# MartinBeseda/FEM-ElastoPlasticity

Hardware: AMD Instinct MI355X
Metric: element*quadpt updates/sec (return-map + K_tan assemble) (higher is better)
Workload: dtype f64; 1 GPU; Plasticity2D_DP strip-footing square, 708x708 cells = 1002528 P1 elements per GPU (BASELINE configs[3]), Drucker-Prager, strain->return map->K_tan CSR values->F per step; element_type=P1, points_per_gpu=1002528, points_total=1002528, elements_total=1002528, nnz_per_gpu=14052388, smooth_points=178150, apex_points=573758, state=bands, route=node, elements_per_gpu=1002528, parallelism=single GPU

## Files before the change

### fem-elastoplasticity_amd/csrc/fep_api.hip

```cpp
#include "fep_common.h"
#include "fep_host.h"
#include "fep_kernels.hip.h"
#include "fep_staging.h"

#include <algorithm>
#include <chrono>
#include <cstdio>
#include <cstdlib>
#include <cstring>
#include <map>
#include <mutex>
#include <new>
#include <thread>
#include <vector>

using namespace fep;

#ifndef FEP_P4_TPB
#define FEP_P4_TPB 256
#define FEP_P4_JS 1
#endif

thread_local int fep_g_last_hip = 0;
#define g_last_hip fep_g_last_hip
// ... 27 lines not shown
    uint16_t *pt_codes = nullptr, *pt_fcodes = nullptr;
    uint4 *pt_fix = nullptr, *pt_ffix = nullptr;
    uint2* pt_fixT = nullptr;
    int64_t n_patch = 0;
#ifdef FEP_ABLATION
    unsigned long long* phase_clk = nullptr;
#endif
    double *Pc = nullptr, *Pf = nullptr;
    bool elem_geo = true;
    MatU matu{};
    int32_t* elem = nullptr;
    double *coords = nullptr, *dh1 = nullptr, *dh2 = nullptr, *wf = nullptr;
    double *dphi1 = nullptr, *dphi2 = nullptr, *weight = nullptr, *det = nullptr;
    double *shear = nullptr, *bulk = nullptr, *eta = nullptr, *c = nullptr;
    int32_t *segptr = nullptr, *perm = nullptr, *iptr = nullptr, *ilist = nullptr;
    uint32_t* meta = nullptr;
    bool p1_lds = false;
    double *geo = nullptr, *xy = nullptr;
    P1Tab p1tab{};
    int32_t *perm2 = nullptr, *ncol = nullptr;
    int32_t *wg_elist = nullptr, *wg_rng = nullptr;
    bool p1_rng = false, p1_pk = false;
    uint2* pk = nullptr;
    int4* tdesc = nullptr;
    int32_t* tstart = nullptr;
    int n_wg_p1 = 0;
    bool p1_fused = false, p1_fused_rng = false;
    bool asm_from_nodes = false;
    bool p1_dma = false;
    int fused_mode = 1;
    int lds_NL = 0;
    int32_t *wg_nlist = nullptr, *wg_nrng = nullptr;
    uint32_t* el_nodes = nullptr;
    unsigned long long* slot_counts = nullptr;
    bool has_orphans = false;
    uint16_t* perm_l = nullptr;
    int tile = 256;
    int gn_tile = 256;
    size_t gn_lds = 0;
    int lds_L = 0, lds_C = 0;
    double *Kc = nullptr, *fe = nullptr;
    double *s_int = nullptr, *ds_int = nullptr;
    uint2* blk_counts = nullptr;
    int n_count_blocks = 0;
    void* hbuf[12] = {};
    size_t hbuf_bytes[12] = {};
    std::vector<int32_t> indptr, indices;
    bool profiling = false;
    std::vector<hipEvent_t> events;
    bool verbose = false;
};

__attribute__((visibility("hidden"))) int fep_set_device(int dev) {
    int n = 0;
    hipError_t e = hipGetDeviceCount(&n);
    if (e != hipSuccess || n <= 0) { g_last_hip = (int)e; (void)hipGetLastError(); return FEP_ENODEV; }
    if (dev < 0 || dev >= n) return FEP_ENODEV;
    e = hipSetDevice(dev);
    if (e != hipSuccess) { g_last_hip = (int)e; (void)hipGetLastError(); return FEP_ENODEV; }
    return FEP_OK;
}

template <class T> static int dmalloc(fep_ctx* c, T** p, int64_t count) {
    *p = nullptr;
    if (count <= 0) count = 1;
    try { c->owned.reserve(c->owned.size() + 1); } catch (...) { return FEP_ENOMEM; }
// ... 353 lines not shown
    fep_ctx* c = nullptr;
    int r;
    try {
        r = ctx_create_impl(c, ctx_out, device_id, elem_type, n_e, n_n, elements_h, coords_h, dhatp1_h, dhatp2_h, wf_h);
    } catch (const std::bad_alloc&) {
        r = FEP_ENOMEM;
    } catch (...) {
        r = FEP_EINVAL;
    }
    if (r != FEP_OK) { if (c) fep_ctx_destroy(c); *ctx_out = nullptr; }
    return r;
}

struct MeshIn {
    const Symbolic& S;
    const int32_t* elem;
    const double *coords, *dh1, *dh2, *wf;
    bool validate;
};

static int setup_p1_node(fep_ctx* c, const MeshIn& in, bool* taken) {
    *taken = false;
    fep_host::P1Options opt;
#ifdef FEP_ABLATION
    if (const char* tl = fep_tune("FEP_P1_TILE")) c->tile = std::atoi(tl) == 128 ? 128 : 256;
    {
        const char* pth = fep_tune("FEP_P1_PATH");
        auto is = [&](const char* v) { return pth && std::strcmp(pth, v) == 0; };
        opt.allow_lds = !is("node_direct");
        opt.allow_rng = !is("node_list");
        opt.allow_pk = !is("node_unpacked");
        opt.allow_fused = !is("node2k");
        if (const char* sg = fep_tune("FEP_P1_SEGS")) opt.max_segs = std::max(1, std::min(std::atoi(sg), fep_host::kSegMax));
    }
#endif
    opt.tile = c->tile;
    fep_host::P1Plan P;
    FEP_TRY(fep_host::build_p1_plan(in.S, c->n_e, c->n_n, in.elem, opt, P));
    if (in.validate) {
        const int bad = fep_host::validate_p1_plan(P, in.S, c->n_e, c->n_n, in.elem);
        if (bad) { std::fprintf(stderr, "[fep] P1 plan fails check %d\n", bad); return FEP_EINVAL; }
    }
#ifndef FEP_ABLATION
    if (!(P.lds && P.pk)) {
        if (c->verbose) std::fprintf(stderr, "[fep] P1 plan without the LDS-staged packed form (lds %d pk %d): element route\n", (int)P.lds, (int)P.pk);
        return FEP_OK;
    }
#endif
    *taken = true;
    c->n_wg_p1 = (int)P.n_wg;
    c->p1_lds = P.lds; c->lds_L = P.L; c->lds_C = P.C; c->p1_rng = P.rng; c->p1_pk = P.pk;
    c->p1_fused = P.fused; c->p1_fused_rng = P.fused_rng; c->lds_NL = P.NL;
#ifdef FEP_ABLATION
    if (const char* am = fep_tune("FEP_P1_ASM")) c->asm_from_nodes = std::strcmp(am, "nodes") == 0;
    if (const char* dm = fep_tune("FEP_P1_DMA")) c->p1_dma = std::strcmp(dm, "0") != 0;
    if (const char* fm = fep_tune("FEP_P1_FUSED"))
        c->fused_mode = std::strcmp(fm, "off") == 0 ? 0 : std::strcmp(fm, "kf") == 0 ? 1 : 2;
#endif
    FEP_TRY(upload(c, &c->perm2, P.perm2.data(), (int64_t)P.perm2.size()));
    FEP_TRY(upload(c, &c->ncol, in.S.ncol.data(), (int64_t)in.S.ncol.size()));
    FEP_TRY(upload(c, &c->tdesc, (const int4*)P.tdesc.data(), (int64_t)P.tdesc.size() / 4));
    if (P.lds) {
        FEP_TRY(upload(c, &c->wg_elist, P.elist_pad.data(), (int64_t)P.elist_pad.size()));
        FEP_TRY(upload(c, &c->perm_l, P.codes_pad.data(), (int64_t)P.codes_pad.size()));
        if (P.rng) FEP_TRY(upload(c, &c->wg_rng, P.rng_tab.data(), (int64_t)P.rng_tab.size()));
        if (P.pk) FEP_TRY(upload(c, &c->pk, (const uint2*)P.pkv.data(), (int64_t)P.pkv.size()));
    }
    if (P.fused) {
        FEP_TRY(upload(c, &c->el_nodes, P.elnodes.data(), (int64_t)P.elnodes.size()));
        if (P.fused_rng) FEP_TRY(upload(c, &c->wg_nrng, P.nrng_tab.data(), (int64_t)P.nrng_tab.size()));
        else FEP_TRY(upload(c, &c->wg_nlist, P.nlist_pad.data(), (int64_t)P.nlist_pad.size()));
        FEP_TRY(dmalloc(c, &c->slot_counts, 256 * 16));
        HIP_TRY(hipMemset(c->slot_counts, 0, 256 * 16 * sizeof(unsigned long long)));
    }
    if (c->verbose)
        std::fprintf(stderr, "[fep] P1 plan: %lld tiles of <= %d blocks in <= %d segment(s), staged elements %lld "
                     "(%.2f per element, <= %d per tile), staged nodes <= %d, codes <= %d; lds %d rng %d pk %d fused %d/%d\n",
                     (long long)P.n_wg, P.tile, P.n_segs, (long long)P.staged_total, (double)P.staged_total / (double)c->n_e,
                     P.L, P.NL, P.C, (int)P.lds, (int)P.rng, (int)P.pk, (int)P.fused, (int)P.fused_rng);
    FEP_TRY(dmalloc(c, &c->geo, 6 * c->n_e));
    for (int a = 0; a < 3; ++a) { c->p1tab.h1[a] = in.dh1[a]; c->p1tab.h2[a] = in.dh2[a]; }
    c->p1tab.wf = in.wf[0];
    c->n_count_blocks = (int)grid_for(c->n_e, kBlock);
    return FEP_OK;
}

#ifdef FEP_ABLATION
static int setup_gen_node(fep_ctx* c, const MeshIn& in, bool* taken) {
    fep_host::GnPlan G;
    fep_host::build_gn_plan(in.S, c->n_p, c->n_q, c->n_e, G);
    *taken = G.ok;
    if (!G.ok) return FEP_OK;
    c->gn_tile = G.tile; c->lds_L = G.L; c->lds_C = G.C; c->gn_lds = G.lds;
    FEP_TRY(upload(c, &c->wg_elist, G.elist_pad.data(), (int64_t)G.elist_pad.size()));
    FEP_TRY(upload(c, &c->perm_l, G.codes_pad.data(), (int64_t)G.codes_pad.size()));
    FEP_TRY(upload(c, &c->ncol, in.S.ncol.data(), (int64_t)in.S.ncol.size()));
    c->n_count_blocks = (int)grid_for(c->n_int, kBlock);
    return FEP_OK;
}
#endif

static void elem_form(fep_ctx* c, bool patch_form) {
    c->elem_geo = elem_geo_default(c->elem_type, patch_form);
#ifdef FEP_ABLATION
    if (const char* ge = fep_tune("FEP_ELEM_GEO")) c->elem_geo = std::strcmp(ge, "0") != 0;
    if (const char* lp = fep_tune("FEP_ELEM_LDS_PAD")) c->lds_pad = std::max(0, std::atoi(lp));
#endif
}

static int setup_patch(fep_ctx* c, const MeshIn& in, bool* taken) {
    *taken = false;
    elem_form(c, true);
// ... 366 lines not shown
}

static int launch_force(fep_ctx* c, hipStream_t st, double* f_out) {
    hipLaunchKernelGGL(force_reduce_kernel, dim3(grid_for(c->n_n, kBlock)), dim3(kBlock), 0, st,
                       c->n_n, c->iptr, c->ilist, c->fe, f_out);
    HIP_TRY(hipGetLastError());
    return FEP_OK;
}

static int launch_fixup(fep_ctx* c, hipStream_t st, double* k_data, double* f_out, unsigned long long* counts_d, bool* counted) {
    const unsigned nb_k = k_data ? grid_for(c->n_open, kBlock) : 0u;
    const unsigned nb_f = f_out ? grid_for(c->n_fopen, kBlock) : 0u;
    const unsigned grid = nb_k + nb_f + (counts_d ? 1u : 0u);
    if (grid == 0) return FEP_OK;
    hipLaunchKernelGGL(fixup_kernel, dim3(grid), dim3(kBlock), 0, st, (int)nb_k, c->n_open, c->pt_fix, c->pt_fixT, c->n_fopen, c->pt_ffix,
                       c->pt_plist, c->Pc, c->Pf, k_data, f_out, c->n_count_blocks, c->blk_counts, counts_d);
    HIP_TRY(hipGetLastError());
    *counted = counts_d != nullptr;
    return FEP_OK;
}

static int launch_p1_node(fep_ctx* c, hipStream_t st, const double* ds, const double* s, double* k_data, double* f_out,
                          unsigned long long* counts_d, bool* counted) {
    if (!((k_data && ds) || (f_out && s))) return FEP_OK;
    if (!k_data) ds = nullptr;
    if (!f_out) s = nullptr;
    const int n_wg = c->n_wg_p1;
    const unsigned grid = 8 * ((n_wg + 7) / 8);
#ifdef FEP_ABLATION
    if (c->p1_fused && c->asm_from_nodes) {
        const size_t lds_stage = (((size_t)c->lds_L * 15 * sizeof(double) + (size_t)c->lds_C * 2 + 15) & ~(size_t)15) +
                                 (size_t)c->lds_NL * 2 * sizeof(double2);
        const size_t lds = std::max(lds_stage, (size_t)c->tile * 3 * sizeof(double2));
        if (c->lds_L > 256 || c->lds_NL > 256) return FEP_ESTATE;
        FEP_TRY(with_bool(c->p1_fused_rng, [&](auto rng) {
            return launch_lds(p1_fused_kernel<false, 256, decltype(rng)::value, 1, 1, true>, grid, 256, lds, kLdsDefault, st,
                              c->n_e, c->lds_L, c->lds_C, c->lds_NL, c->perm_l, c->wg_elist, (const int4*)c->wg_rng,
                              c->wg_nlist, (const int4*)c->wg_nrng, c->el_nodes, c->pk, c->tdesc, c->xy, c->p1tab,
                              (const double*)nullptr, make_e0(nullptr), (const double*)nullptr, c->shear, c->bulk, c->eta,
                              c->c, c->matu, (double*)nullptr, (double*)nullptr, (double*)nullptr, (uint8_t*)nullptr,
                              k_data, f_out, n_wg, (unsigned long long*)nullptr, ds, s, c->n_count_blocks, c->blk_counts, counts_d);
        }));
        *counted = counts_d != nullptr;
        return FEP_OK;
    }
    if (!c->p1_lds) {
        hipLaunchKernelGGL(p1_node_kernel, dim3(grid_for(c->n_blk, kBlock)), dim3(kBlock), 0, st,
                           c->n_blk, c->n_e, c->segptr, c->perm2, c->meta, c->ncol, c->geo, ds, s, k_data, f_out);
        HIP_TRY(hipGetLastError());
        return FEP_OK;
    }
#else
    if (!c->p1_lds) return FEP_ESTATE;
#endif
    const size_t lds = std::max((size_t)c->lds_L * 15 * sizeof(double) + (size_t)c->lds_C * sizeof(uint16_t),
                                (size_t)c->tile * 3 * sizeof(double2));
    if (c->verbose) {
        static bool once = false;
        if (!once) {
            once = true;
            std::fprintf(stderr, "[fep] p1 assembly kernel: %d tiles of <= %d blocks, staged elements <= %d, codes <= %d, "
                         "LDS %zu bytes per workgroup\n", n_wg, c->tile, c->lds_L, c->lds_C, lds);
        }
    }
    FEP_TRY(with_ablation_bool<false>(c->tile == 128, [&](auto t128) {
        constexpr int TPB = decltype(t128)::value ? 128 : 256;
        if (c->lds_L > TPB) return FEP_ESTATE;
        return with_bool(c->p1_rng, [&](auto rng) {
            return with_ablation_bool<true>(c->p1_pk, [&](auto pk) {
                return launch_lds(p1_node_lds_kernel<TPB, decltype(rng)::value, 1, decltype(pk)::value>, grid, TPB, lds,
                                  kLdsDefault, st, c->n_e, c->lds_L, c->lds_C, c->segptr, c->perm_l, c->meta, c->ncol,
// ... 31 lines not shown
    FEP_TRY(with_type(c->elem_type, [&](auto et) {
        using ET = decltype(et);
        if constexpr (ET::type == FEP_P1 || ET::type == FEP_P4) return FEP_EINVAL;
        else return with_bool(c->gn_tile == 256, [&](auto t256) {
            constexpr int TPB = decltype(t256)::value ? 256 : 128;
            return launch_lds(node_lds_kernel<ET::NP, ET::NQ, TPB>, grid, TPB, c->gn_lds, kLdsNodeLds, st, c->n_blk, c->n_e,
                              c->lds_L, c->lds_C, c->segptr, c->perm_l, c->meta, c->ncol, c->wg_elist, c->elem, c->xy,
                              c->dh1, c->dh2, c->wf, k_data ? ds : nullptr, f_out ? s : nullptr, k_data, f_out, n_wg,
                              c->n_count_blocks, c->blk_counts, counts_d);
        });
    }));
    *counted = counts_d != nullptr;
    return FEP_OK;
}
#endif

static int launch_p1_fused(fep_ctx* c, hipStream_t st, const double* u, E0 e0, const double* ep, double* eout, double* s,
                           double* ds, uint8_t* indp, double* k_data, double* f_out, unsigned long long* counts_d) {
    const bool dma = c->p1_dma;
    const size_t Cp = dma ? ((size_t)c->lds_C + 127) & ~(size_t)127 : (size_t)c->lds_C;
    const size_t NLp = dma ? ((size_t)c->lds_NL + 63) & ~(size_t)63 : (size_t)c->lds_NL;
    const size_t lds_stage = (((size_t)c->lds_L * 15 * sizeof(double) + Cp * 2 + 15) & ~(size_t)15) + NLp * 2 * sizeof(double2);
    const size_t lds = std::max(lds_stage, (size_t)c->tile * 3 * sizeof(double2));
    const int n_wg = c->n_wg_p1;
    const unsigned grid = 8 * ((n_wg + 7) / 8);
    if (c->lds_L > c->tile || c->lds_NL > c->tile) return FEP_ESTATE;
    const bool full = eout || s || ds || indp;
    FEP_TRY(with_ablation_bool<false>(full, [&](auto full_c) {
        return with_bool(c->p1_fused_rng, [&](auto rng) {
            return with_ablation_bool<false>(dma, [&](auto dma_c) {
                return with_ablation_bool<false>(c->tile == 128, [&](auto t128) {
                    constexpr int TPB = decltype(t128)::value ? 128 : 256;
                    return launch_lds(p1_fused_kernel<decltype(full_c)::value, TPB, decltype(rng)::value, 1, 1, false, decltype(dma_c)::value>,
                                      grid, TPB, lds, kLdsDefault, st, c->n_e, c->lds_L, c->lds_C, c->lds_NL, c->perm_l,
                                      c->wg_elist, (const int4*)c->wg_rng, c->wg_nlist, (const int4*)c->wg_nrng, c->el_nodes,
                                      c->pk, c->tdesc, c->xy, c->p1tab, u, e0, ep, c->shear, c->bulk, c->eta, c->c, c->matu,
                                      eout, s, ds, indp, k_data, f_out, n_wg,
                                      counts_d ? c->slot_counts : (unsigned long long*)nullptr, (const double*)nullptr,
                                      (const double*)nullptr, 0, (const uint2*)nullptr, (unsigned long long*)nullptr);
                });
            });
        });
    }));
    if (counts_d) {
        hipLaunchKernelGGL(counts_finalize_kernel, dim3(1), dim3(256), 0, st, c->slot_counts, counts_d);
        HIP_TRY(hipGetLastError());
    }
    return FEP_OK;
}

static int launch_assembly(fep_ctx* c, hipStream_t st, const double* ds, const double* s, double* k_data, double* f_out,
                           unsigned long long* counts_d, bool* counted, bool* f_due) {
    *counted = *f_due = false;
    if (c->route == Route::P1Node) return launch_p1_node(c, st, ds, s, k_data, f_out, counts_d, counted);
#ifdef FEP_ABLATION
    if (c->route == Route::GenNode) return launch_gn_node(c, st, ds, s, k_data, f_out, counts_d, counted);
#endif
    if (c->route == Route::Patch) return launch_fixup(c, st, k_data, f_out, counts_d, counted);
    return launch_reduce(c, st, k_data, f_out, counts_d, counted, f_due);
}

extern "C" int fep_step_dev(fep_ctx* c, void* stream, const double* u_d, const double* e0_h,
                            double* ep_prev_d, int accept, double* e_out_d, double* s_d, double* ds_d,
                            uint8_t* ind_p_d, double* k_data_d, double* f_out_d, int64_t* counts_d) {
    if (!c || !u_d) return FEP_EINVAL;
    if (!fep_aligned16(u_d) || !fep_aligned16(f_out_d) || !fep_aligned16(k_data_d)) return FEP_EINVAL;
    if (!c->have_materials) return FEP_ESTATE;
    FEP_TRY(fep_set_device(c->device));
    hipStream_t st = (hipStream_t)stream;
// ... 384 lines not shown
```

### fem-elastoplasticity_amd/csrc/fep_host.h

```cpp
#pragma once
#include <algorithm>
#include <atomic>
#include <cstdint>
#include <cstdlib>
#include <cstring>
#include <exception>
#include <new>
#include <system_error>
#include <thread>
#include <utility>
#include <vector>

#include "../../include/fep.h"

namespace fep_host {

struct U2 { uint32_t x, y; };

inline int worker_count() {
    if (const char* e = std::getenv("FEP_HOST_THREADS")) { const int v = std::atoi(e); if (v >= 1) return std::min(v, 64); }
    return (int)std::max(1u, std::min(16u, std::thread::hardware_concurrency()));
}

template <class F> void parallel_chunks(int64_t n, F&& f) {
    const int nw = (int)std::max<int64_t>(1, std::min<int64_t>(worker_count(), n));
    std::vector<std::thread> th;
    th.reserve(nw);
    std::vector<int> inline_chunks;
    std::vector<std::exception_ptr> err((size_t)nw);
    auto guarded = [&f, &err](int64_t lo, int64_t hi, int w) {
        try { f(lo, hi, w); } catch (...) { err[(size_t)w] = std::current_exception(); }
    };
    for (int w = 1; w < nw; ++w) {
        const int64_t lo = n * w / nw, hi = n * (w + 1) / nw;
        try { th.emplace_back([&guarded, lo, hi, w]() { guarded(lo, hi, w); }); }
        catch (const std::system_error&) { inline_chunks.push_back(w); }
    }
    guarded(0, n / nw, 0);
    for (int w : inline_chunks) guarded(n * w / nw, n * (w + 1) / nw, w);
    for (auto& t : th) t.join();
    for (const std::exception_ptr& e : err)
        if (e) std::rethrow_exception(e);
// ... 67 lines not shown
                    const int64_t blk = S.nptr[n] + slot;
                    S.ncol[blk] = buf[i].first;
                    S.meta[blk] = ((uint32_t)deg[n] << 16) | (buf[i].first == (int32_t)n ? 0x8000u : 0u) | (uint32_t)slot;
                    S.segptr[blk] = (int32_t)pos;
                }
                S.perm[pos++] = buf[i].second;
            }
        }
    });
    S.segptr[n_blk] = (int32_t)n_contrib;
    return FEP_OK;
}

inline int row_tiles(const Symbolic& S, int64_t n_n, int tile, std::vector<int32_t>& tstart) {
    tstart.assign(1, 0);
    for (int64_t n = 0, cur = 0; n < n_n; ++n) {
        const int64_t d = S.nptr[n + 1] - S.nptr[n];
        if (d > tile) return FEP_ERANGE;
        if (cur + d > tile) { tstart.push_back(S.nptr[n]); cur = 0; }
        cur += d;
    }
    tstart.push_back(S.nptr[n_n]);
    return FEP_OK;
}

constexpr int kSegMax = 4;
constexpr int kDescInts = 4 * (1 + kSegMax);

struct P1Options {
    int tile = 256;
    int max_segs = 2;
    int staged_cap = 128;
    bool allow_lds = true, allow_rng = true, allow_pk = true, allow_fused = true;
};

struct P1Plan {
    int tile = 256, n_segs = 1;
    int64_t n_wg = 0, staged_total = 0, staged_nodes_total = 0;
    std::vector<int32_t> tdesc;
    std::vector<int32_t> perm2;
    bool lds = false, rng = false, pk = false, fused = false, fused_rng = false;
    int L = 0, C = 0, NL = 0;
    std::vector<int32_t> elist_pad, rng_tab, nlist_pad, nrng_tab;
    std::vector<uint16_t> codes_pad;
    std::vector<U2> pkv;
    std::vector<uint32_t> elnodes;
};

struct Tile { int nseg = 0; int32_t fb[kSegMax] = {}, nb[kSegMax] = {}, fn[kSegMax] = {}, nn[kSegMax] = {}; };

inline int make_tiles(const Symbolic& S, int64_t n_n, int tile, int max_segs, std::vector<Tile>& tiles) {
    tiles.clear();
    max_segs = std::max(1, std::min(max_segs, kSegMax));
    std::vector<uint8_t> assigned((size_t)n_n, 0);
    for (int64_t n = 0; n < n_n; ++n) assigned[n] = S.nptr[n + 1] == S.nptr[n];
    std::vector<int32_t> nbrs;
    int64_t p = 0;
    while (true) {
        while (p < n_n && assigned[p]) ++p;
        if (p >= n_n) break;
        Tile t;
        int total_nodes = 0, total_blocks = 0;
        int64_t start = p;
        for (int s = 0; s < max_segs; ++s) {
            const int seg_budget = std::min((tile - total_blocks + (max_segs - s) - 1) / (max_segs - s),
                                            max_segs > 1 ? tile / max_segs + 8 : tile);
            int64_t n = start;
            int blocks = 0;
            while (n < n_n && !assigned[n] && blocks + (S.nptr[n + 1] - S.nptr[n]) <= seg_budget && total_nodes + (int)(n - start) < 255) {
                blocks += S.nptr[n + 1] - S.nptr[n];
                ++n;
            }
            if (n == start) {
                if (s > 0) break;
                if (S.nptr[n + 1] - S.nptr[n] > tile) return FEP_ERANGE;
                blocks = S.nptr[n + 1] - S.nptr[n];
                ++n;
            }
            t.fb[s] = S.nptr[start]; t.nb[s] = blocks; t.fn[s] = (int32_t)start; t.nn[s] = (int32_t)(n - start);
// ... 9 lines not shown
            nbrs.erase(std::unique(nbrs.begin(), nbrs.end()), nbrs.end());
            size_t best = 0, best_len = 0;
            for (size_t i = 0; i < nbrs.size();) {
                size_t j = i + 1;
                while (j < nbrs.size() && nbrs[j] == nbrs[j - 1] + 1) ++j;
                if (j - i > best_len) { best_len = j - i; best = i; }
                i = j;
            }
            if (best_len < 2) break;
            start = nbrs[best];
            {
                int64_t lo = start;
                int gap = 0;
                while (lo > 0 && !assigned[lo - 1] && gap < 32) { --lo; ++gap; }
                if (gap < 32) start = lo;
            }
        }
        tiles.push_back(t);
    }
    return FEP_OK;
}

inline void runs_of(const std::vector<int32_t>& l, int32_t* d , bool& fits) {
    int nr = 0, cum = 0;
    for (size_t i = 0; i < l.size();) {
        size_t j = i + 1;
        while (j < l.size() && l[j] == l[j - 1] + 1) ++j;
        if (nr == 8) { fits = false; break; }
        cum += (int)(j - i);
        d[2 * nr] = l[i]; d[2 * nr + 1] = cum;
        ++nr; i = j;
    }
    for (; nr < 8; ++nr) { d[2 * nr] = l.empty() ? 0 : l[0]; d[2 * nr + 1] = cum; }
}

inline int build_p1_plan_segs(const Symbolic& S, int64_t n_e, int64_t n_n, const int32_t* elem, const P1Options& opt,
                              int max_segs, P1Plan& P) {
    P = P1Plan();
    P.tile = opt.tile;
    const int TILE = opt.tile;
    if (n_e >= (int64_t)1 << 27) return FEP_ERANGE;
    const int64_t n_blk = (int64_t)S.ncol.size();
    P.perm2.resize(S.perm.size());
    for (size_t i = 0; i < S.perm.size(); ++i) {
        const int64_t code = S.perm[i];
        const int64_t ab = code / n_e, e = code - ab * n_e;
        P.perm2[i] = (int32_t)((e << 4) | ((ab / 3) << 2) | (ab % 3));
    }
    std::vector<Tile> tiles;
    const int r = make_tiles(S, n_n, TILE, max_segs, tiles);
    if (r != FEP_OK) return r;
    if (max_segs > 1 && opt.staged_cap > 0) {
        std::vector<int32_t> count(tiles.size(), 0);
        parallel_chunks((int64_t)tiles.size(), [&](int64_t lo, int64_t hi, int) {
            std::vector<int32_t> l;
            for (int64_t g = lo; g < hi; ++g) {
                const Tile& t = tiles[g];
                if (t.nseg < 2) continue;
                l.clear();
                for (int s = 0; s < t.nseg; ++s)
                    for (int32_t c = S.segptr[t.fb[s]]; c < S.segptr[t.fb[s] + t.nb[s]]; ++c) l.push_back(P.perm2[c] >> 4);
                std::sort(l.begin(), l.end());
                count[g] = (int32_t)(std::unique(l.begin(), l.end()) - l.begin());
            }
        });
        std::vector<Tile> split;
// ... 112 lines not shown
                const int32_t* d = P.tdesc.data() + g * kDescInts;
                const int nb = d[1];
                if (d[2] > 255) { pk_bad[g] = 1; continue; }
                order.resize(nb); blk.resize(nb); node_of.resize(nb); off.resize(nb);
                int k = 0, node_base = 0, o = 0;
                for (int s = 0; s < t.nseg; ++s) {
                    for (int32_t n = t.fn[s]; n < t.fn[s] + t.nn[s]; ++n)
                        for (int32_t b = S.nptr[n]; b < S.nptr[n + 1]; ++b) {
                            blk[k] = b; node_of[k] = node_base + (n - t.fn[s]); off[k] = o;
                            o += S.segptr[b + 1] - S.segptr[b];
                            ++k;
                        }
                    node_base += t.nn[s];
                }
                if (k != nb) { pk_bad[g] = 1; continue; }
                for (int i = 0; i < nb; ++i) order[i] = i;
                std::stable_sort(order.begin(), order.end(), [&](int x, int y) {
                    return S.segptr[blk[x] + 1] - S.segptr[blk[x]] > S.segptr[blk[y] + 1] - S.segptr[blk[y]];
                });
                for (int lane = 0; lane < nb; ++lane) {
                    const int kk = order[lane];
                    const int32_t b = blk[kk];
                    const uint32_t mt = S.meta[b];
                    const uint32_t len = (uint32_t)(S.segptr[b + 1] - S.segptr[b]), deg = mt >> 16, slot = mt & 0x7fffu;
                    const uint32_t diag = (mt >> 15) & 1u;
                    if (len > 15 || deg > 255 || slot > 255 || off[kk] > 2047) { pk_bad[g] = 1; break; }
                    P.pkv[(size_t)d[0] + lane] = U2{(uint32_t)off[kk] | (len << 11) | (deg << 15) | (slot << 23) | (diag << 31),
                                                    (uint32_t)kk | ((uint32_t)node_of[kk] << 8)};
                }
            }
        });
    for (int64_t g = 0; g < n_wg && pk_ok; ++g) pk_ok = !pk_bad[g];
    P.pk = pk_ok;
    if (!pk_ok) { P.pkv.clear(); return FEP_OK; }
    if (!opt.allow_fused) return FEP_OK;
    std::vector<std::vector<int32_t>> nlists(n_wg);
    P.elnodes.assign((size_t)(n_wg * LP), 0u);
    std::vector<uint8_t> nbad((size_t)n_wg, 0);
    parallel_chunks(n_wg, [&](int64_t lo, int64_t hi, int) {
        for (int64_t g = lo; g < hi; ++g) {
            const std::vector<int32_t>& l = lists[g];
            std::vector<int32_t>& nl = nlists[g];
            nl.reserve(3 * l.size());
            for (int32_t e : l)
                for (int a = 0; a < 3; ++a) nl.push_back(elem[(int64_t)a * n_e + e]);
            std::sort(nl.begin(), nl.end());
            nl.erase(std::unique(nl.begin(), nl.end()), nl.end());
            if (nl.size() > 1023) { nbad[g] = 1; continue; }
            for (size_t i = 0; i < l.size(); ++i) {
                uint32_t word = 0u;
                for (int a = 0; a < 3; ++a) {
                    const int32_t nd = elem[(int64_t)a * n_e + l[i]];
                    word |= (uint32_t)(std::lower_bound(nl.begin(), nl.end(), nd) - nl.begin()) << (10 * a);
                }
                P.elnodes[(size_t)(g * LP) + i] = word;
            }
            for (size_t i = l.size(); i < (size_t)LP; ++i) P.elnodes[(size_t)(g * LP) + i] = P.elnodes[(size_t)(g * LP)];
        }
    });
    size_t nlmax = 0;
    for (int64_t g = 0; g < n_wg; ++g) {
        if (nbad[g]) { P.elnodes.clear(); return FEP_OK; }
        nlmax = std::max(nlmax, nlists[g].size());
        P.staged_nodes_total += (int64_t)nlists[g].size();
    }
    if (nlmax == 0 || nlmax > (size_t)TILE) { P.elnodes.clear(); return FEP_OK; }
    for (int64_t g = 0; g < n_wg; ++g) {
        for (int32_t i = 0; i < n_own[g]; ++i) P.elnodes[(size_t)(g * LP) + i] |= 1u << 30;
        P.tdesc[(size_t)g * kDescInts + 2] |= n_own[g] << 8;
    }
    const int64_t NLP = (int64_t)((nlmax + 1) & ~(size_t)1);
    P.NL = (int)NLP;
    P.nlist_pad.assign((size_t)(n_wg * NLP), 0);
    P.nrng_tab.assign((size_t)n_wg * 16, 0);
    bool nfits = P.rng;
    for (int64_t g = 0; g < n_wg; ++g) {
        const std::vector<int32_t>& nl = nlists[g];
        std::fill(P.nlist_pad.begin() + g * NLP, P.nlist_pad.begin() + (g + 1) * NLP, nl[0]);
        std::copy(nl.begin(), nl.end(), P.nlist_pad.begin() + g * NLP);
        if (nfits) runs_of(nl, P.nrng_tab.data() + g * 16, nfits);
    }
    for (int64_t g = 0; g < n_wg; ++g) P.tdesc[(size_t)g * kDescInts + 3] |= (int32_t)(nlists[g].size() << 16);
    P.fused_rng = nfits;
    const size_t lds_f = (((size_t)P.L * 15 * sizeof(double) + (size_t)P.C * 2 + 15) & ~(size_t)15) + (size_t)NLP * 32;
    P.fused = lds_f <= 96 * 1024;
    if (!P.fused) P.elnodes.clear();
    return FEP_OK;
}

inline int build_p1_plan(const Symbolic& S, int64_t n_e, int64_t n_n, const int32_t* elem, const P1Options& opt, P1Plan& P) {
    int r = build_p1_plan_segs(S, n_e, n_n, elem, opt, 1, P);
    if (r != FEP_OK || opt.max_segs <= 1 || !P.lds || !P.pk) return r;
    P1Plan Q;
    r = build_p1_plan_segs(S, n_e, n_n, elem, opt, opt.max_segs, Q);
    if (r == FEP_OK && Q.lds && Q.pk && (Q.fused || !P.fused) && (Q.rng || !P.rng) && (Q.fused_rng || !P.fused_rng) &&
        Q.staged_total * 100 <= P.staged_total * 95) P = std::move(Q);
    return FEP_OK;
}

inline int validate_p1_plan(const P1Plan& P, const Symbolic& S, int64_t n_e, int64_t n_n, const int32_t* elem) {
    const int64_t n_blk = (int64_t)S.ncol.size();
    if ((int64_t)P.tdesc.size() != P.n_wg * kDescInts) return 1;
    std::vector<uint8_t> seen((size_t)n_blk, 0);
    std::vector<int> owners((size_t)n_e, 0);
    int64_t pk_base = 0;
    for (int64_t g = 0; g < P.n_wg; ++g) {
        const int32_t* d = P.tdesc.data() + g * kDescInts;
        const int nseg = d[3] & 15, n_staged = (d[3] >> 4) & 4095, n_staged_nodes = (d[3] >> 16) & 4095;
        const int nn_desc = d[2] & 255, n_own = d[2] >> 8;
        if (d[0] != pk_base || nseg < 1 || nseg > kSegMax || d[1] > P.tile || d[1] < 1 || n_own > n_staged) return 2;
        int nb = 0, nn = 0;
        for (int s = 0; s < nseg; ++s) {
            const int32_t fb = d[4 + 4 * s], sb = d[5 + 4 * s], fn = d[6 + 4 * s], sn = d[7 + 4 * s];
            if (fn < 0 || fn + sn > n_n || sn < 1 || S.nptr[fn] != fb || S.nptr[fn + sn] != fb + sb) return 3;
            for (int32_t b = fb; b < fb + sb; ++b) { if (seen[b]) return 4; seen[b] = 1; }
            nb += sb; nn += sn;
        }
        if (nb != d[1] || nn != nn_desc) return 5;
        pk_base += nb;
        if (!P.lds) continue;
        const int32_t* el = P.elist_pad.data() + g * P.L;
        const int n_list = n_staged;
        if (n_list < 1 || n_list > P.L) return 18;
        for (int i = 0; i < P.L; ++i) {
            if (el[i] < 0 || el[i] >= n_e) return 6;
            if (i >= n_list && el[i] != el[0]) return 18;
        }
        {
            std::vector<int32_t> srt(el, el + n_list);
            std::sort(srt.begin(), srt.end());
            if (std::adjacent_find(srt.begin(), srt.end()) != srt.end()) return 18;
            if (P.fused)
                for (int i = 1; i < n_list; ++i)
                    if (i != n_own && el[i] <= el[i - 1]) return 18;
        }
        if (P.rng) {
            const int32_t* r = P.rng_tab.data() + g * 16;
            for (int i = 0; i < P.L; ++i) {
                int e = r[0] + i;
                for (int k = 1; k < 8; ++k) e = i >= r[2 * k - 1] ? r[2 * k] + (i - r[2 * k - 1]) : e;
                e = i < r[15] ? e : r[0];
                if (e != el[i]) return 7;
            }
// ... 2 lines not shown
            std::vector<uint8_t> lane_blk((size_t)nb, 0);
            for (int lane = 0; lane < nb; ++lane) {
                const U2 w = P.pkv[(size_t)d[0] + lane];
                const int beg = (int)(w.x & 2047u), len = (int)((w.x >> 11) & 15u), deg = (int)((w.x >> 15) & 255u);
                const int slot = (int)((w.x >> 23) & 255u), blk = (int)(w.y & 255u), nod = (int)((w.y >> 8) & 255u);
                if (beg + len > P.C || blk >= nb || nod >= nn || lane_blk[blk]) return 8;
                lane_blk[blk] = 1;
                const int rel = 4 * blk - 2 * slot;
                if (rel < 0 || (rel >> 1) + deg + 1 > 2 * nb || slot >= deg) return 9;
                for (int c = beg; c < beg + len; ++c) {
                    const unsigned code = P.codes_pad[(size_t)g * P.C + c];
                    if ((int)(code >> 4) >= n_list || ((code >> 2) & 3) > 2 || (code & 3) > 2) return 10;
                }
            }
        }
        if (P.fused) {
            const int32_t* nl = P.nlist_pad.data() + g * P.NL;
            int n_nl = 1;
            for (int i = 0; i < P.NL; ++i) {
                if (nl[i] < 0 || nl[i] >= n_n) return 11;
                if (i > 0 && nl[i] > nl[i - 1]) n_nl = i + 1;
            }
            if (n_nl != n_staged_nodes) return 19;
            if (P.fused_rng) {
                const int32_t* r = P.nrng_tab.data() + g * 16;
                for (int i = 0; i < P.NL; ++i) {
                    int n = r[0] + i;
                    for (int k = 1; k < 8; ++k) n = i >= r[2 * k - 1] ? r[2 * k] + (i - r[2 * k - 1]) : n;
                    n = i < r[15] ? n : r[0];
                    if (n != nl[i]) return 12;
                }
            }
            for (int i = 0; i < P.L; ++i) {
                const uint32_t w = P.elnodes[(size_t)g * P.L + i];
                for (int a = 0; a < 3; ++a) {
                    const int loc = (int)((w >> (10 * a)) & 1023u);
                    if (loc >= P.NL || nl[loc] != elem[(int64_t)a * n_e + el[i]]) return 13;
                }
                if (((w >> 30) & 1u) != (i < n_own ? 1u : 0u)) return 14;
                if (i < n_own) owners[el[i]]++;
            }
        }
    }
    if (pk_base != n_blk) return 15;
    for (int64_t b = 0; b < n_blk; ++b) if (!seen[b]) return 16;
    if (P.fused) for (int64_t e = 0; e < n_e; ++e) if (owners[e] != 1) return 17;
    return 0;
}

struct GnPlan {
    bool ok = false;
    int tile = 256, L = 0, C = 0;
    size_t lds = 0;
    std::vector<int32_t> elist_pad;
    std::vector<uint16_t> codes_pad;
};

inline void build_gn_plan(const Symbolic& S, int n_p, int n_q, int64_t n_e, GnPlan& G) {
    const int64_t n_blk = (int64_t)S.ncol.size();
    for (int TILE : {256, 128}) {
        const int64_t n_wg = (n_blk + TILE - 1) / TILE;
        std::vector<std::vector<int32_t>> lists(n_wg);
        std::vector<uint16_t> perm_l(S.perm.size());
        std::vector<uint8_t> bad((size_t)n_wg, 0);
        parallel_chunks(n_wg, [&](int64_t lo, int64_t hi, int) {
            for (int64_t g = lo; g < hi; ++g) {
                const int64_t b0 = g * TILE, b1 = std::min<int64_t>(n_blk, b0 + TILE);
                const int32_t t0 = S.segptr[b0], t1 = S.segptr[b1];
                std::vector<int32_t>& l = lists[g];
                l.reserve(t1 - t0);
                for (int32_t t = t0; t < t1; ++t) l.push_back((int32_t)(S.perm[t] % n_e));
                std::sort(l.begin(), l.end());
                l.erase(std::unique(l.begin(), l.end()), l.end());
                if (l.size() > 256) { bad[g] = 1; continue; }
                for (int32_t t = t0; t < t1; ++t) {
                    const int64_t ab = S.perm[t] / n_e, e = S.perm[t] % n_e;
                    const int32_t loc = (int32_t)(std::lower_bound(l.begin(), l.end(), (int32_t)e) - l.begin());
// ... 782 lines not shown
```

### fem-elastoplasticity_amd/csrc/fep_kernels.hip.h

```cpp
#pragma once
#include <hip/hip_runtime.h>
#include <stdint.h>

namespace fep {

constexpr int kBlock = 256;

#ifndef FEP_P2_FMA
#define FEP_P2_FMA 1
#endif

__device__ __forceinline__ void lds_barrier() { asm volatile("s_waitcnt lgkmcnt(0)\n\ts_barrier" ::: "memory"); }

__device__ __forceinline__ int dp_return_map(const double e[3], const double z[4], double p[4],
                                             double G, double K, double eta, double c, bool accept,
                                             double s[4], double d[6]) {
    const double I3 = 1.0 / 3.0;
    const double DD = 1.0 - 1.0 / 3.0;
    const double RS2 = 1.4142135623730951;
    const double Et0 = (e[0] + z[0]) - p[0];
    const double Et1 = (e[1] + z[1]) - p[1];
    const double Et2 = (e[2] + z[2]) - p[2];
    const double Et3 = (0.0 + z[3]) - p[3];
    const double tr = Et0 + Et1 + Et3;
// ... 1183 lines not shown
        out2[rel >> 1] = make_double2(k00, k01);
        out2[(rel >> 1) + (int)deg] = make_double2(k10, k11);
    }
    double2* fo2 = out2 + 2 * TPB;
    if (PK) { if (want_f) fo2[fnode_k] = make_double2(f0, f1); }
    __syncthreads();
    store_tile_outputs<TPB>(td, out2, fo2, data, (PK && S != nullptr) ? F : nullptr);
    if (!PK && want_f) *reinterpret_cast<double2*>(F + 2 * (int64_t)ncol_sb) = make_double2(f0, f1);
}

template <bool FULL, int TPB, bool RNG, int EPT, int NPT, bool FROM_DS = false, bool DMA = false>
__global__ void __launch_bounds__(TPB, (!FULL && EPT == 1) ? 8 : 1)
p1_fused_kernel(int64_t n_e, int L, int C, int NL,
                const uint16_t* __restrict__ perm_l, const int32_t* __restrict__ wg_elist, const int4* __restrict__ rng,
                const int32_t* __restrict__ wg_nlist, const int4* __restrict__ nrng,
                const uint32_t* __restrict__ el_nodes, const uint2* __restrict__ pk, const int4* __restrict__ tdesc,
                const double* __restrict__ xy, P1Tab tab, const double* __restrict__ U, E0 e0,
                const double* __restrict__ ep,
                const double* __restrict__ shear, const double* __restrict__ bulk,
                const double* __restrict__ eta, const double* __restrict__ cc, MatU mu,
                double* __restrict__ Eout, double* __restrict__ S, double* __restrict__ DS, uint8_t* __restrict__ indp,
                double* __restrict__ data, double* __restrict__ F, int n_wg, unsigned long long* __restrict__ slot_counts,
                const double* __restrict__ DSin, const double* __restrict__ Sin,
                int n_count_blocks, const uint2* __restrict__ blk_counts, unsigned long long* __restrict__ counts_out) {
    static_assert(!(FULL && FROM_DS), "the assembly-only form has no point outputs");
    extern __shared__ __attribute__((aligned(16))) double rec[];
    if (FROM_DS && counts_out != nullptr && blockIdx.x == 0) sum_block_counts(n_count_blocks, blk_counts, counts_out);
    __shared__ unsigned int sc[2];
    const int chunk = (n_wg + 7) >> 3;
    const int wg = (int)(blockIdx.x & 7) * chunk + (int)(blockIdx.x >> 3);
    if (wg >= n_wg) return;
    const TileDesc td = load_tile_desc(tdesc, wg);
    const int nb = td.nb;
    const int64_t sb = (int64_t)td.pk_base + threadIdx.x;
    const bool live = (int)threadIdx.x < nb;
    constexpr int CWPT = 2;
    if (threadIdx.x == 0) { sc[0] = 0u; sc[1] = 0u; }
    int64_t el[EPT];
    int64_t nd[NPT];
    if (RNG) {
        const int4* d = rng + (int64_t)wg * 4;
        const int4 d0 = d[0], d1 = d[1], d2 = d[2], d3 = d[3];
        const int st[8] = {d0.x, d0.z, d1.x, d1.z, d2.x, d2.z, d3.x, d3.z};
        const int cu[8] = {d0.y, d0.w, d1.y, d1.w, d2.y, d2.w, d3.y, d3.w};
#pragma unroll
        for (int r = 0; r < EPT; ++r) {
            const int i = r * TPB + (int)threadIdx.x;
            int e = st[0] + i;
#pragma unroll
            for (int k = 1; k < 8; ++k) e = i >= cu[k - 1] ? st[k] + (i - cu[k - 1]) : e;
            el[r] = i < cu[7] ? e : st[0];
        }
        const int4* dn = nrng + (int64_t)wg * 4;
        const int4 n0 = dn[0], n1 = dn[1], n2 = dn[2], n3 = dn[3];
        const int sn[8] = {n0.x, n0.z, n1.x, n1.z, n2.x, n2.z, n3.x, n3.z};
        const int cn[8] = {n0.y, n0.w, n1.y, n1.w, n2.y, n2.w, n3.y, n3.w};
#pragma unroll
        for (int r = 0; r < NPT; ++r) {
            const int i = r * TPB + (int)threadIdx.x;
            int n = sn[0] + i;
#pragma unroll
            for (int k = 1; k < 8; ++k) n = i >= cn[k - 1] ? sn[k] + (i - cn[k - 1]) : n;
            nd[r] = i < cn[7] ? n : sn[0];
        }
    } else {
#pragma unroll
// ... 3 lines not shown
        }
#pragma unroll
        for (int r = 0; r < NPT; ++r) {
            const int i = r * TPB + (int)threadIdx.x;
            nd[r] = wg_nlist[(int64_t)wg * NL + (i < NL ? i : 0)];
        }
    }
    const int n_el = td.n_el, n_nd = td.n_nd;
    const int Cp = DMA ? (C + 127) & ~127 : C, NLp = DMA ? (NL + 63) & ~63 : NL;
    uint16_t* codes = reinterpret_cast<uint16_t*>(rec + 15 * L);
    uint32_t* codes32 = reinterpret_cast<uint32_t*>(rec + 15 * L);
    double2* lxy = reinterpret_cast<double2*>(reinterpret_cast<char*>(rec) + (((size_t)15 * L * 8 + (size_t)Cp * 2 + 15) & ~(size_t)15));
    double2* lu = lxy + NLp;
    double2 nxy[NPT], nu[NPT];
#pragma unroll
    for (int r = 0; r < NPT; ++r) {
        if (r * TPB + (int)(threadIdx.x & ~63u) >= n_nd) continue;
        if (DMA) {
            glds16(xy + 2 * nd[r], lxy + r * TPB + (int)(threadIdx.x & ~63u));
            if (!FROM_DS) glds16(U + 2 * nd[r], lu + r * TPB + (int)(threadIdx.x & ~63u));
        } else {
            nxy[r] = *reinterpret_cast<const double2*>(xy + 2 * nd[r]);
            if (!FROM_DS) nu[r] = *reinterpret_cast<const double2*>(U + 2 * nd[r]);
        }
    }
    uint32_t enw[EPT];
    double pv[EPT][4], mv[EPT][4];
    double dvi[EPT][6], svi[EPT][3];
#pragma unroll
    for (int r = 0; r < EPT; ++r) {
        if (r * TPB + (int)(threadIdx.x & ~63u) >= n_el) continue;
        const int i = r * TPB + (int)threadIdx.x;
        const int64_t e = el[r];
        enw[r] = el_nodes[(int64_t)wg * L + (i < L ? i : 0)];
        if (FROM_DS) {
            if (DSin) {
                dvi[r][0] = DSin[e]; dvi[r][1] = DSin[n_e + e]; dvi[r][2] = DSin[2 * n_e + e];
                dvi[r][3] = DSin[4 * n_e + e]; dvi[r][4] = DSin[5 * n_e + e]; dvi[r][5] = DSin[8 * n_e + e];
            }
            if (Sin) { svi[r][0] = Sin[e]; svi[r][1] = Sin[n_e + e]; svi[r][2] = Sin[2 * n_e + e]; }
        } else {
            if (ep) { pv[r][0] = ep[e]; pv[r][1] = ep[n_e + e]; pv[r][2] = ep[2 * n_e + e]; pv[r][3] = ep[3 * n_e + e]; }
            else { pv[r][0] = 0.0; pv[r][1] = 0.0; pv[r][2] = 0.0; pv[r][3] = 0.0; }
            if (!mu.on) { mv[r][0] = shear[e]; mv[r][1] = bulk[e]; mv[r][2] = eta[e]; mv[r][3] = cc[e]; }
        }
    }
    const uint2 w2 = live ? pk[sb] : make_uint2(0u, 0u);
    const int CW = C >> 1;
    const uint32_t* codes_w = reinterpret_cast<const uint32_t*>(perm_l) + (int64_t)wg * CW;
    uint32_t cd[CWPT];
#pragma unroll
    for (int r = 0; r < CWPT; ++r) {
        const int i = r * TPB + (int)threadIdx.x;
        cd[r] = 0u;
        if (r * TPB + (int)(threadIdx.x & ~63u) < CW) {
            if (DMA) glds4(codes_w + (i < CW ? i : 0), codes32 + r * TPB + (int)(threadIdx.x & ~63u));
            else cd[r] = codes_w[i < CW ? i : 0];
        }
    }
    if (!DMA) {
#pragma unroll
        for (int r = 0; r < NPT; ++r) {
            const int i = r * TPB + (int)threadIdx.x;
            if (i < n_nd) { lxy[i] = nxy[r]; if (!FROM_DS) lu[i] = nu[r]; }
        }
#pragma unroll
        for (int q = 0; q < CWPT; ++q) {
            const int ci = q * TPB + (int)threadIdx.x;
            if (ci < CW) codes32[ci] = cd[q];
        }
    }
    __syncthreads();
    unsigned int n_sm = 0u, n_ap = 0u;
#pragma unroll
    for (int r = 0; r < EPT; ++r) {
        const int i = r * TPB + (int)threadIdx.x;
        int branch = 0;
        bool own = false;
        if (i < n_el) {
            const uint32_t wv = enw[r];
            const int64_t e = el[r];
            own = i < td.n_own;
// ... 291 lines not shown
```

Measured before the change: 11.14 billion updates/s.

## Deduplicate identical per-tile P1 tables into shared equivalence classes

Hashes each tile's packed block words, LDS codes and element-node words, groups identical tiles into classes, and stores only one copy of those tables per class. The fused kernel then indexes the tables by class, taken from a rewritten tile descriptor, instead of by workgroup. On a structured mesh many tiles should share tables, so the point is to cut global/L2 traffic for these metadata tables and improve cache hit rates. In exchange it adds host-side hashing at setup and extra validation checks.

```diff
diff --git a/fem-elastoplasticity_amd/csrc/fep_api.hip b/fem-elastoplasticity_amd/csrc/fep_api.hip
--- a/fem-elastoplasticity_amd/csrc/fep_api.hip
+++ b/fem-elastoplasticity_amd/csrc/fep_api.hip
@@ -83,6 +83,9 @@
     int lds_NL = 0;
     int32_t *wg_nlist = nullptr, *wg_nrng = nullptr;
     uint32_t* el_nodes = nullptr;
+    int4* tdesc_c = nullptr;
+    uint16_t* perm_c = nullptr;
+    uint2* pk_c = nullptr;
     unsigned long long* slot_counts = nullptr;
     bool has_orphans = false;
     uint16_t* perm_l = nullptr;
@@ -502,6 +505,7 @@
         opt.allow_pk = !is("node_unpacked");
         opt.allow_fused = !is("node2k");
         if (const char* sg = fep_tune("FEP_P1_SEGS")) opt.max_segs = std::max(1, std::min(std::atoi(sg), fep_host::kSegMax));
+        if (const char* sh = fep_tune("FEP_P1_SHARE")) opt.share_tables = std::strcmp(sh, "0") != 0;
     }
 #endif
     opt.tile = c->tile;
@@ -538,6 +542,9 @@
     }
     if (P.fused) {
         FEP_TRY(upload(c, &c->el_nodes, P.elnodes.data(), (int64_t)P.elnodes.size()));
+        FEP_TRY(upload(c, &c->tdesc_c, (const int4*)P.tdesc_c.data(), (int64_t)P.tdesc_c.size() / 4));
+        FEP_TRY(upload(c, &c->perm_c, P.codes_c.data(), (int64_t)P.codes_c.size()));
+        FEP_TRY(upload(c, &c->pk_c, (const uint2*)P.pkv_c.data(), (int64_t)P.pkv_c.size()));
         if (P.fused_rng) FEP_TRY(upload(c, &c->wg_nrng, P.nrng_tab.data(), (int64_t)P.nrng_tab.size()));
         else FEP_TRY(upload(c, &c->wg_nlist, P.nlist_pad.data(), (int64_t)P.nlist_pad.size()));
         FEP_TRY(dmalloc(c, &c->slot_counts, 256 * 16));
@@ -545,9 +552,11 @@
     }
     if (c->verbose)
         std::fprintf(stderr, "[fep] P1 plan: %lld tiles of <= %d blocks in <= %d segment(s), staged elements %lld "
-                     "(%.2f per element, <= %d per tile), staged nodes <= %d, codes <= %d; lds %d rng %d pk %d fused %d/%d\n",
+                     "(%.2f per element, <= %d per tile), staged nodes <= %d, codes <= %d; lds %d rng %d pk %d fused %d/%d; "
+                     "%lld table set(s) of the one-kernel step, %zu bytes\n",
                      (long long)P.n_wg, P.tile, P.n_segs, (long long)P.staged_total, (double)P.staged_total / (double)c->n_e,
-                     P.L, P.NL, P.C, (int)P.lds, (int)P.rng, (int)P.pk, (int)P.fused, (int)P.fused_rng);
+                     P.L, P.NL, P.C, (int)P.lds, (int)P.rng, (int)P.pk, (int)P.fused, (int)P.fused_rng, (long long)P.n_class,
+                     P.pkv_c.size() * sizeof(fep_host::U2) + P.codes_c.size() * sizeof(uint16_t) + P.elnodes.size() * sizeof(uint32_t));
     FEP_TRY(dmalloc(c, &c->geo, 6 * c->n_e));
     for (int a = 0; a < 3; ++a) { c->p1tab.h1[a] = in.dh1[a]; c->p1tab.h2[a] = in.dh2[a]; }
     c->p1tab.wf = in.wf[0];
@@ -980,11 +989,11 @@
         const size_t lds_stage = (((size_t)c->lds_L * 15 * sizeof(double) + (size_t)c->lds_C * 2 + 15) & ~(size_t)15) +
                                  (size_t)c->lds_NL * 2 * sizeof(double2);
         const size_t lds = std::max(lds_stage, (size_t)c->tile * 3 * sizeof(double2));
-        if (c->lds_L > 256 || c->lds_NL > 256) return FEP_ESTATE;
+        if (c->lds_L > 256 || c->lds_NL > 256 || c->tile != 256) return FEP_ESTATE;
         FEP_TRY(with_bool(c->p1_fused_rng, [&](auto rng) {
             return launch_lds(p1_fused_kernel<false, 256, decltype(rng)::value, 1, 1, true>, grid, 256, lds, kLdsDefault, st,
-                              c->n_e, c->lds_L, c->lds_C, c->lds_NL, c->perm_l, c->wg_elist, (const int4*)c->wg_rng,
-                              c->wg_nlist, (const int4*)c->wg_nrng, c->el_nodes, c->pk, c->tdesc, c->xy, c->p1tab,
+                              c->n_e, c->lds_L, c->lds_C, c->lds_NL, c->perm_c, c->wg_elist, (const int4*)c->wg_rng,
+                              c->wg_nlist, (const int4*)c->wg_nrng, c->el_nodes, c->pk_c, c->tdesc_c, c->xy, c->p1tab,
                               (const double*)nullptr, make_e0(nullptr), (const double*)nullptr, c->shear, c->bulk, c->eta,
                               c->c, c->matu, (double*)nullptr, (double*)nullptr, (double*)nullptr, (uint8_t*)nullptr,
                               k_data, f_out, n_wg, (unsigned long long*)nullptr, ds, s, c->n_count_blocks, c->blk_counts, counts_d);
@@ -1082,9 +1091,9 @@
                 return with_ablation_bool<false>(c->tile == 128, [&](auto t128) {
                     constexpr int TPB = decltype(t128)::value ? 128 : 256;
                     return launch_lds(p1_fused_kernel<decltype(full_c)::value, TPB, decltype(rng)::value, 1, 1, false, decltype(dma_c)::value>,
-                                      grid, TPB, lds, kLdsDefault, st, c->n_e, c->lds_L, c->lds_C, c->lds_NL, c->perm_l,
+                                      grid, TPB, lds, kLdsDefault, st, c->n_e, c->lds_L, c->lds_C, c->lds_NL, c->perm_c,
                                       c->wg_elist, (const int4*)c->wg_rng, c->wg_nlist, (const int4*)c->wg_nrng, c->el_nodes,
-                                      c->pk, c->tdesc, c->xy, c->p1tab, u, e0, ep, c->shear, c->bulk, c->eta, c->c, c->matu,
+                                      c->pk_c, c->tdesc_c, c->xy, c->p1tab, u, e0, ep, c->shear, c->bulk, c->eta, c->c, c->matu,
                                       eout, s, ds, indp, k_data, f_out, n_wg,
                                       counts_d ? c->slot_counts : (unsigned long long*)nullptr, (const double*)nullptr,
                                       (const double*)nullptr, 0, (const uint2*)nullptr, (unsigned long long*)nullptr);
diff --git a/fem-elastoplasticity_amd/csrc/fep_host.h b/fem-elastoplasticity_amd/csrc/fep_host.h
--- a/fem-elastoplasticity_amd/csrc/fep_host.h
+++ b/fem-elastoplasticity_amd/csrc/fep_host.h
@@ -1,6 +1,7 @@
 #pragma once
 #include <algorithm>
 #include <atomic>
+#include <climits>
 #include <cstdint>
 #include <cstdlib>
 #include <cstring>
@@ -8,6 +9,7 @@
 #include <new>
 #include <system_error>
 #include <thread>
+#include <unordered_map>
 #include <utility>
 #include <vector>
 
@@ -141,6 +143,7 @@
     int max_segs = 2;
     int staged_cap = 128;
     bool allow_lds = true, allow_rng = true, allow_pk = true, allow_fused = true;
+    bool share_tables = true;
 };
 
 struct P1Plan {
@@ -154,6 +157,11 @@
     std::vector<uint16_t> codes_pad;
     std::vector<U2> pkv;
     std::vector<uint32_t> elnodes;
+    int64_t n_class = 0;
+    std::vector<int32_t> tclass;
+    std::vector<int32_t> tdesc_c;
+    std::vector<U2> pkv_c;
+    std::vector<uint16_t> codes_c;
 };
 
 struct Tile { int nseg = 0; int32_t fb[kSegMax] = {}, nb[kSegMax] = {}, fn[kSegMax] = {}, nn[kSegMax] = {}; };
@@ -229,6 +237,70 @@
         ++nr; i = j;
     }
     for (; nr < 8; ++nr) { d[2 * nr] = l.empty() ? 0 : l[0]; d[2 * nr + 1] = cum; }
+}
+
+inline int share_p1_tables(P1Plan& P, bool share) {
+    const int64_t n_wg = P.n_wg;
+    const size_t T = (size_t)P.tile, C = (size_t)P.C, L = (size_t)P.L;
+    P.tclass.clear(); P.tdesc_c.clear(); P.pkv_c.clear(); P.codes_c.clear(); P.n_class = 0;
+    if (P.elnodes.empty()) return FEP_OK;
+    auto desc = [&](int64_t g) { return P.tdesc.data() + g * kDescInts; };
+    auto same = [&](int64_t g, int64_t h) {
+        const int32_t *dg = desc(g), *dh = desc(h);
+        return dg[1] == dh[1] &&
+               std::memcmp(&P.pkv[(size_t)dg[0]], &P.pkv[(size_t)dh[0]], (size_t)dg[1] * sizeof(U2)) == 0 &&
+               std::memcmp(&P.codes_pad[(size_t)g * C], &P.codes_pad[(size_t)h * C], C * sizeof(uint16_t)) == 0 &&
+               std::memcmp(&P.elnodes[(size_t)g * L], &P.elnodes[(size_t)h * L], L * sizeof(uint32_t)) == 0;
+    };
+    P.tclass.assign((size_t)n_wg, 0);
+    std::vector<int64_t> rep;
+    if (!share) {
+        rep.resize((size_t)n_wg);
+        for (int64_t g = 0; g < n_wg; ++g) { rep[(size_t)g] = g; P.tclass[(size_t)g] = (int32_t)g; }
+    } else {
+        std::vector<uint64_t> hash((size_t)n_wg);
+        parallel_chunks(n_wg, [&](int64_t lo, int64_t hi, int) {
+            for (int64_t g = lo; g < hi; ++g) {
+                uint64_t h = 1469598103934665603ull;
+                auto mix = [&](const void* p, size_t n) {
+                    const unsigned char* b = static_cast<const unsigned char*>(p);
+                    for (size_t i = 0; i < n; ++i) h = (h ^ b[i]) * 1099511628211ull;
+                };
+                const int32_t* d = desc(g);
+                mix(&d[1], sizeof(int32_t));
+                mix(&P.pkv[(size_t)d[0]], (size_t)d[1] * sizeof(U2));
+                mix(&P.codes_pad[(size_t)g * C], C * sizeof(uint16_t));
+                mix(&P.elnodes[(size_t)g * L], L * sizeof(uint32_t));
+                hash[(size_t)g] = h;
+            }
+        });
+        std::unordered_map<uint64_t, std::vector<int32_t>> by_hash;
+        for (int64_t g = 0; g < n_wg; ++g) {
+            std::vector<int32_t>& cand = by_hash[hash[(size_t)g]];
+            int32_t cls = -1;
+            for (int32_t c : cand)
+                if (same(g, rep[(size_t)c])) { cls = c; break; }
+            if (cls < 0) { cls = (int32_t)rep.size(); rep.push_back(g); cand.push_back(cls); }
+            P.tclass[(size_t)g] = cls;
+        }
+    }
+    const size_t n_class = rep.size();
+    if (n_class * T > (size_t)INT32_MAX) return FEP_ERANGE;
+    P.codes_c.assign(n_class * C, 0);
+    P.pkv_c.assign(n_class * T, U2{0u, 0u});
+    std::vector<uint32_t> elnodes(n_class * L);
+    for (size_t c = 0; c < n_class; ++c) {
+        const int64_t g = rep[c];
+        const int32_t* d = desc(g);
+        std::copy_n(&P.codes_pad[(size_t)g * C], C, &P.codes_c[c * C]);
+        std::copy_n(&P.pkv[(size_t)d[0]], (size_t)d[1], &P.pkv_c[c * T]);
+        std::copy_n(&P.elnodes[(size_t)g * L], L, &elnodes[c * L]);
+    }
+    P.elnodes.swap(elnodes);
+    P.n_class = (int64_t)n_class;
+    P.tdesc_c = P.tdesc;
+    for (int64_t g = 0; g < n_wg; ++g) P.tdesc_c[(size_t)g * kDescInts] = (int32_t)((size_t)P.tclass[(size_t)g] * T);
+    return FEP_OK;
 }
 
 inline int build_p1_plan_segs(const Symbolic& S, int64_t n_e, int64_t n_n, const int32_t* elem, const P1Options& opt,
@@ -407,8 +479,8 @@
         });
     for (int64_t g = 0; g < n_wg && pk_ok; ++g) pk_ok = !pk_bad[g];
     P.pk = pk_ok;
-    if (!pk_ok) { P.pkv.clear(); return FEP_OK; }
-    if (!opt.allow_fused) return FEP_OK;
+    if (!pk_ok) { P.pkv.clear(); return share_p1_tables(P, opt.share_tables); }
+    if (!opt.allow_fused) return share_p1_tables(P, opt.share_tables);
     std::vector<std::vector<int32_t>> nlists(n_wg);
     P.elnodes.assign((size_t)(n_wg * LP), 0u);
     std::vector<uint8_t> nbad((size_t)n_wg, 0);
@@ -435,11 +507,11 @@
     });
     size_t nlmax = 0;
     for (int64_t g = 0; g < n_wg; ++g) {
-        if (nbad[g]) { P.elnodes.clear(); return FEP_OK; }
+        if (nbad[g]) { P.elnodes.clear(); return share_p1_tables(P, opt.share_tables); }
         nlmax = std::max(nlmax, nlists[g].size());
         P.staged_nodes_total += (int64_t)nlists[g].size();
     }
-    if (nlmax == 0 || nlmax > (size_t)TILE) { P.elnodes.clear(); return FEP_OK; }
+    if (nlmax == 0 || nlmax > (size_t)TILE) { P.elnodes.clear(); return share_p1_tables(P, opt.share_tables); }
     for (int64_t g = 0; g < n_wg; ++g) {
         for (int32_t i = 0; i < n_own[g]; ++i) P.elnodes[(size_t)(g * LP) + i] |= 1u << 30;
         P.tdesc[(size_t)g * kDescInts + 2] |= n_own[g] << 8;
@@ -460,7 +532,7 @@
     const size_t lds_f = (((size_t)P.L * 15 * sizeof(double) + (size_t)P.C * 2 + 15) & ~(size_t)15) + (size_t)NLP * 32;
     P.fused = lds_f <= 96 * 1024;
     if (!P.fused) P.elnodes.clear();
-    return FEP_OK;
+    return share_p1_tables(P, opt.share_tables);
 }
 
 inline int build_p1_plan(const Symbolic& S, int64_t n_e, int64_t n_n, const int32_t* elem, const P1Options& opt, P1Plan& P) {
@@ -479,11 +551,27 @@
     std::vector<uint8_t> seen((size_t)n_blk, 0);
     std::vector<int> owners((size_t)n_e, 0);
     int64_t pk_base = 0;
+    if (P.fused) {
+        if ((int64_t)P.tclass.size() != P.n_wg || P.n_class < 1 || P.n_class > P.n_wg ||
+            P.n_class * P.tile > (int64_t)INT32_MAX || P.tdesc_c.size() != P.tdesc.size()) return 20;
+        if ((int64_t)P.codes_c.size() != P.n_class * P.C || (int64_t)P.pkv_c.size() != P.n_class * P.tile ||
+            (int64_t)P.elnodes.size() != P.n_class * P.L) return 20;
+    }
+    int64_t next_class = 0;
     for (int64_t g = 0; g < P.n_wg; ++g) {
         const int32_t* d = P.tdesc.data() + g * kDescInts;
         const int nseg = d[3] & 15, n_staged = (d[3] >> 4) & 4095, n_staged_nodes = (d[3] >> 16) & 4095;
         const int nn_desc = d[2] & 255, n_own = d[2] >> 8;
         if (d[0] != pk_base || nseg < 1 || nseg > kSegMax || d[1] > P.tile || d[1] < 1 || n_own > n_staged) return 2;
+        const int64_t cls = P.fused ? P.tclass[(size_t)g] : 0;
+        if (P.fused) {
+            const int32_t* dc = P.tdesc_c.data() + g * kDescInts;
+            if (cls < 0 || cls > next_class || cls >= P.n_class || dc[0] != cls * P.tile) return 21;
+            next_class = std::max(next_class, cls + 1);
+            if (std::memcmp(dc + 1, d + 1, (kDescInts - 1) * sizeof(int32_t)) != 0) return 21;
+            if (std::memcmp(&P.pkv_c[(size_t)dc[0]], &P.pkv[(size_t)d[0]], (size_t)d[1] * sizeof(U2)) != 0 ||
+                std::memcmp(&P.codes_c[(size_t)cls * P.C], &P.codes_pad[(size_t)g * P.C], (size_t)P.C * sizeof(uint16_t)) != 0) return 23;
+        }
         int nb = 0, nn = 0;
         for (int s = 0; s < nseg; ++s) {
             const int32_t fb = d[4 + 4 * s], sb = d[5 + 4 * s], fn = d[6 + 4 * s], sn = d[7 + 4 * s];
@@ -552,7 +640,7 @@
                 }
             }
             for (int i = 0; i < P.L; ++i) {
-                const uint32_t w = P.elnodes[(size_t)g * P.L + i];
+                const uint32_t w = P.elnodes[(size_t)cls * P.L + i];
                 for (int a = 0; a < 3; ++a) {
                     const int loc = (int)((w >> (10 * a)) & 1023u);
                     if (loc >= P.NL || nl[loc] != elem[(int64_t)a * n_e + el[i]]) return 13;
@@ -563,6 +651,7 @@
         }
     }
     if (pk_base != n_blk) return 15;
+    if (P.fused && next_class != P.n_class) return 22;
     for (int64_t b = 0; b < n_blk; ++b) if (!seen[b]) return 16;
     if (P.fused) for (int64_t e = 0; e < n_e; ++e) if (owners[e] != 1) return 17;
     return 0;
diff --git a/fem-elastoplasticity_amd/csrc/fep_kernels.hip.h b/fem-elastoplasticity_amd/csrc/fep_kernels.hip.h
--- a/fem-elastoplasticity_amd/csrc/fep_kernels.hip.h
+++ b/fem-elastoplasticity_amd/csrc/fep_kernels.hip.h
@@ -1239,6 +1239,7 @@
     if (wg >= n_wg) return;
     const TileDesc td = load_tile_desc(tdesc, wg);
     const int nb = td.nb;
+    const int64_t tcls = (uint32_t)td.pk_base / TPB;
     const int64_t sb = (int64_t)td.pk_base + threadIdx.x;
     const bool live = (int)threadIdx.x < nb;
     constexpr int CWPT = 2;
@@ -1308,7 +1309,7 @@
         if (r * TPB + (int)(threadIdx.x & ~63u) >= n_el) continue;
         const int i = r * TPB + (int)threadIdx.x;
         const int64_t e = el[r];
-        enw[r] = el_nodes[(int64_t)wg * L + (i < L ? i : 0)];
+        enw[r] = el_nodes[tcls * L + (i < L ? i : 0)];
         if (FROM_DS) {
             if (DSin) {
                 dvi[r][0] = DSin[e]; dvi[r][1] = DSin[n_e + e]; dvi[r][2] = DSin[2 * n_e + e];
@@ -1323,7 +1324,7 @@
     }
     const uint2 w2 = live ? pk[sb] : make_uint2(0u, 0u);
     const int CW = C >> 1;
-    const uint32_t* codes_w = reinterpret_cast<const uint32_t*>(perm_l) + (int64_t)wg * CW;
+    const uint32_t* codes_w = reinterpret_cast<const uint32_t*>(perm_l) + tcls * CW;
     uint32_t cd[CWPT];
 #pragma unroll
     for (int r = 0; r < CWPT; ++r) {
```

New measurement: 11.24 billion updates/s (median of 4 runs). About the same (+0.9%).
